# TravisWheelerLab/BATH

Hardware: AMD Instinct MI355X
Metric: DP Gcells/s + residues/s through bathsearch pipeline at 1/2/4/8 MI355X (higher is better)
Workload: dtype u8/i16 integer scores (SSV: exact binary16), f32 Forward

## Files before the change

### bath_amd/__init__.py

```python
import ctypes as C
import os
import subprocess

import numpy as np

_HERE = os.path.dirname(os.path.abspath(__file__))
_ROOT = os.path.dirname(_HERE)
LIB_PATH = os.environ.get("BATH_HIP_LIBRARY") or os.path.join(_HERE, "libbathhip.so")

OK, ERANGE, ENORESULT = 0, 16, 19
KP, K, NEVPARAM = 29, 20, 8
LOGSUM_TABLE, LOGSUM_EXACT, LOGSUM_TABLE_SERIAL, LOGSUM_CONTEXT = 0, 1, 2, 3
LOGSUM_ODDS = 4
ENSEMBLE_SERIAL, ENSEMBLE_STREAMS_HOST, ENSEMBLE_STREAMS_DEVICE = 0, 1, 2
ENSEMBLE_MODES = {"serial": ENSEMBLE_SERIAL, "streams": ENSEMBLE_STREAMS_HOST, "device": ENSEMBLE_STREAMS_DEVICE}
ENS_SAMPLES = 200
ENS_OK, ENS_IMPOSSIBLE, ENS_STEP_CAP, ENS_SEG_OVERFLOW = 0, 1, 2, 3
ENS_REGION_OK, ENS_REGION_NO_TRACES = 0, 1

DNA_SYMS = "ACGT-RYMKSWHBVDN*~"
AMINO_SYMS = "ACDEFGHIKLMNPQRSTVWY-BJZOUX*~"


class BathError(RuntimeError):
# ... 134 lines not shown


class Fs5Result(C.Structure):
    _fields_ = [("fwdsc", C.c_float), ("bcksc", C.c_float), ("oasc", C.c_float), ("null2", C.c_float * KP)]


_vp, _u8p, _f32p, _i32p, _i64p = C.c_void_p, C.POINTER(C.c_uint8), C.POINTER(C.c_float), C.POINTER(C.c_int32), C.POINTER(C.c_int64)
ABI = {
    "bath_hmmfile_count": (C.c_int, [C.c_char_p]),
    "bath_hmmfile_read": (C.c_int, [C.c_char_p, C.c_int, C.POINTER(C.POINTER(_Hmm))]),
    "bath_hmm_destroy": (None, [C.POINTER(_Hmm)]),
    "bath_gencode_basic": (C.c_int, [C.c_int, _u8p]),
    "bath_profile_config": (C.c_int, [C.POINTER(_Hmm), C.c_int, C.POINTER(C.POINTER(_Profile))]),
    "bath_profile_destroy": (None, [C.POINTER(_Profile)]),
    "bath_fs_profile_config": (C.c_int, [C.POINTER(_Hmm), _u8p, C.c_int, C.c_int, C.POINTER(C.POINTER(_FsProfile))]),
    "bath_fs_profile_destroy": (None, [C.POINTER(_FsProfile)]),
    "bath_hip_init": (C.c_int, [C.c_int, C.POINTER(_vp)]),
    "bath_hip_finalize": (None, [_vp]),
    "bath_hip_last_error": (C.c_char_p, [_vp]),
    "bath_hip_synchronize": (C.c_int, [_vp]),
    "bath_hip_stream": (_vp, [_vp]),
    "bath_hip_set_fs_strict": (C.c_int, [_vp, C.c_int]),
    "bath_hip_set_fs_serial": (C.c_int, [_vp, C.c_int]),
    "bath_hip_set_fs_odds": (C.c_int, [_vp, C.c_int]),
    "bath_hip_set_fs5_odds": (C.c_int, [_vp, C.c_int]),
    "bath_hip_set_fs_ensemble": (C.c_int, [_vp, C.c_int]),
    "bath_hip_fs_ensemble_counters": (C.c_int, [_vp, _i64p, _i64p, _i64p]),
    "bath_hip_set_std_ensemble": (C.c_int, [_vp, C.c_int]),
    "bath_hip_std_ensemble_counters": (C.c_int, [_vp, _i64p, _i64p, _i64p]),
    "bath_hip_std_region_ensembles": (C.c_int, [_vp, _vp, _vp, _i32p, C.c_uint32, _i32p, _i32p, _i32p, C.c_int64, _i64p, _i32p, _f32p, C.c_int64, _i64p]),
    "bath_selftest_std_ensemble": (C.c_int, [C.c_int, C.c_int, _f32p, _f32p, C.c_float, C.c_float, C.c_float, _u8p, C.c_int, _f32p, _f32p, C.c_uint32, _i32p, _i32p,
                                             _i32p, C.c_int, _i32p, _f32p, _i32p, C.c_int, _i32p]),
    "bath_selftest_std_ens_walk": (C.c_int, [C.c_int, _f32p, C.c_float, C.c_float, C.c_float, C.c_int, _f32p, _f32p, C.c_uint32, _i32p, _i32p, C.c_int, _i32p]),
    "bath_hip_fs5_region_ensembles": (C.c_int, [_vp, _vp, _vp, C.c_uint32, _i32p, _i32p, _i32p, C.c_int64, _i64p, _i32p, C.c_int64, _i64p]),
    "bath_selftest_fs_ensemble_seeded": (C.c_int, [C.c_int, _f32p, C.c_float, C.c_float, C.c_float, C.c_int, C.c_int, _f32p, _f32p, C.c_uint32, _i32p, C.c_int, _i32p]),
    "bath_selftest_fs_ensemble_streams": (C.c_int, [C.c_int, _f32p, C.c_float, C.c_float, C.c_float, C.c_int, C.c_int, _f32p, _f32p, C.c_uint32,
                                                    _i32p, _i32p, _i32p, C.c_int, _i32p, _i32p, C.c_int, _i32p]),
    "bath_selftest_rng_jump": (C.c_int, [C.c_uint32, C.c_uint64, C.POINTER(C.c_uint32)]),
    "bath_selftest_ens_explog": (C.c_int, [C.c_int, _f32p, _f32p, _f32p]),
    "bath_hip_trim": (C.c_int, [_vp]),
    "bath_hip_kernel_times": (C.c_int, [_vp, C.c_int, C.POINTER(KernelTime)]),
    "bath_hip_oprofile_convert": (C.c_int, [_vp, C.POINTER(_Profile), C.POINTER(_vp)]),
    "bath_hip_oprofile_destroy": (None, [_vp]),
    "bath_hip_oprofile_M": (C.c_int, [_vp]),
    "bath_hip_oprofile_scalars": (C.c_int, [_vp, C.c_int, C.POINTER(OProfileScalars)]),
    "bath_hip_oprofile_get_ssv_scores": (C.c_int, [_vp, _u8p]),
# ... 248 lines not shown

    def set_fs5_odds(self, on=True):
        self._check(lib().bath_hip_set_fs5_odds(self._h, 1 if on else 0), "set_fs5_odds")

    def set_fs_ensemble(self, mode):
        self._check(lib().bath_hip_set_fs_ensemble(self._h, ENSEMBLE_MODES.get(mode, mode)), "set_fs_ensemble")

    def fs_ensemble_counters(self):
        a, b, c = C.c_int64(0), C.c_int64(0), C.c_int64(0)
        self._check(lib().bath_hip_fs_ensemble_counters(self._h, C.byref(a), C.byref(b), C.byref(c)), "fs_ensemble_counters")
        return {"bound_fallbacks": a.value, "overflow_fallbacks": b.value, "matrix_bytes_kept": c.value}

    def set_std_ensemble(self, mode):
        self._check(lib().bath_hip_set_std_ensemble(self._h, ENSEMBLE_MODES.get(mode, mode)), "set_std_ensemble")

    def std_ensemble_counters(self):
        a, b, c = C.c_int64(0), C.c_int64(0), C.c_int64(0)
        self._check(lib().bath_hip_std_ensemble_counters(self._h, C.byref(a), C.byref(b), C.byref(c)), "std_ensemble_counters")
        return {"serial_fallbacks": a.value, "twin_fallbacks": b.value, "kernel_regions": c.value}

    def set_fs_serial(self, on):
        self._check(lib().bath_hip_set_fs_serial(self._h, -1 if on is None else (1 if on else 0)), "set_fs_serial")

    @property
    def stream(self):
        return lib().bath_hip_stream(self._h)

    def close(self):
        if getattr(self, "_h", None):
            lib().bath_hip_finalize(self._h)
            self._h = None

    def __del__(self):
        self.close()


class OProfile:

    def __init__(self, ctx, gm):
        h = _vp()
        ctx._check(lib().bath_hip_oprofile_convert(ctx._h, gm._p, C.byref(h)), "oprofile_convert")
        self.ctx, self._h, self.M, self.gm = ctx, h, gm.M, gm
        hmm = getattr(gm, "hmm", None)
        if hmm is not None and hmm.consensus:
            ctx._check(lib().bath_hip_oprofile_set_consensus(h, hmm.consensus.encode()), "oprofile_set_consensus")

# ... 845 lines not shown
```

### bath_amd/csrc/bath_common.hpp

```cpp
#pragma once
#include <set>
#include <atomic>
#include <hip/hip_runtime.h>

#include <cstdint>
#include <chrono>
#include <cstdio>
#include <cstdlib>
#include <cstring>
#include <condition_variable>
#include <functional>
#include <mutex>
#include <string>
#include <thread>
#include <vector>

#include "bath_hip.h"
#include "bath_tilings.hpp"

namespace bath {

inline hipError_t allow_max_lds(const void *fn) {
  static std::mutex mu;
  static std::set<std::pair<int, const void *>> done;
// ... 115 lines not shown

struct bath_hip_ctx;
namespace bath {
extern std::atomic<int> g_ctx_total, g_ctx_internal;
inline int host_contexts() { return g_ctx_total.load() - g_ctx_internal.load(); }
inline void mark_internal(bath_hip_ctx *c);
}
struct bath_hip_ctx {
  int device = 0;
  hipStream_t stream = nullptr;
  hipStream_t tail_stream = nullptr;
  hipStream_t side_stream = nullptr;
  hipEvent_t ev_fork = nullptr, ev_join = nullptr;
  hipStream_t copy_stream = nullptr;
  hipDeviceProp_t prop{};
  int fs_strict = 1;
  int fs_odds = 0;
  int fs5_odds = 0;
  int fs_ensemble = 0;
  std::atomic<int64_t> fs_ens_bound_fallbacks{0}, fs_ens_overflow_fallbacks{0}, fs_ens_bytes_kept{0};
  int std_ensemble = 0;
  std::atomic<int64_t> std_ens_serial_fallbacks{0}, std_ens_twin_fallbacks{0}, std_ens_kernel_regions{0};
  int fs_serial = -1;
  uint64_t tabs_uid = 0;
  const void *tabs_ptr = nullptr;
  uint64_t fsw_pad_uid = 0;
  int orf_tables_id = -1;
  std::string err;
  void set_error(const std::string &m) { err = m; }
  bath::DevBuf scratch[62];
  bath::HostBuf stage[12];
  template <class T> int stage_upload(int slot, void *dst, const T *src, size_t n, hipStream_t s) {
    if (stage[slot].reserve(n * sizeof(T) + 64) != hipSuccess) { set_error("cannot allocate page-locked staging memory"); return BATH_EFAIL; }
    std::memcpy(stage[slot].p, src, n * sizeof(T));
    if (hipMemcpyAsync(dst, stage[slot].p, n * sizeof(T), hipMemcpyHostToDevice, s) != hipSuccess) { set_error("staging upload failed"); return BATH_EFAIL; }
    return BATH_OK;
  }
  bath::HostBuf pinned[4];
  bath::HostBuf results_pinned;
  bath_orf_result *d_records = nullptr;
  int64_t n_records = 0;
  std::vector<bath_orf> orfs;
  std::vector<bath_fs_window> fs_windows;
  bool keep_fwd_rows = false;
  const float *fwd_rows_kept = nullptr;
  const int64_t *fwd_rows_off = nullptr;
// ... 171 lines not shown
```

### bath_amd/csrc/bath_pipeline.hip

```cpp
#include <algorithm>
#include <cmath>
#include <cstring>
#include <cstdlib>
#include <map>
#include <thread>

#include "bath_common.hpp"
#include "bath_kernels.hpp"
#include "bath_launch.hpp"
#include "host_model.hpp"

using namespace bath;

namespace bath {

static const double kLog2 = 0.69314718055994529;

enum { FLAG_VIT_RUN = 1, FLAG_HAS_WIN = 2 };

struct Counters {
  int cand_count, todo_msv, todo_vit, todo_ssvb, todo_vit2, todo_fwd, win_count, overflow;
  int todo_lb, pad_;
  unsigned long long n_orfs, orf_res;
  unsigned long long n_past_msv, n_past_bias, n_past_vit, n_past_fwd;
  unsigned long long pos_past_msv, pos_past_bias, pos_past_vit, pos_past_fwd;
  unsigned long long res_vit, res_fwd;
  unsigned long long res_seen;
};

struct Params {
  double F1, F2, F3, F4;
  int do_bias, fs_pipe, minlen;
  float evparam[BATH_NEVPARAM];
};

template <int NR, int G>
__global__ __launch_bounds__(256, NR <= 76 ? 4 : 1) void ssv_orf_kernel(const uint8_t *__restrict__ aa, const OrfRec *__restrict__ orfs, const int *__restrict__ n_orfs_dev,
                                                      SeqView dna, const int16_t *__restrict__ cost_tab, int row_bytes,
                                                      const int16_t *__restrict__ emit_thresh, int thresh_max,
                                                      Cand cand, int cand_cap, Counters *__restrict__ ctr, int chunk) {
  extern __shared__ __attribute__((aligned(16))) char lds[];
  if (chunk > 0 && (int64_t)blockIdx.x * (blockDim.x >> 6) * chunk * (64 / G) >= (int64_t)*n_orfs_dev) return;
  {
    const int n32 = kSsvRows * row_bytes / 4;
    const uint32_t *src = reinterpret_cast<const uint32_t *>(cost_tab);
// ... 284 lines not shown
  local_compo_finish(compo, bgf, eo);
}
__device__ void local_compo_finish(float *compo, const float *bgf, float *eo) {
  float sum = 0.f, cc = 0.f;
  for (int x = 0; x < 20; x++) { const float y = compo[x] - cc; const float t = sum + y; cc = (t - sum) - y; sum = t; }
  if (sum != 0.0f) for (int x = 0; x < 20; x++) compo[x] /= sum;
  else for (int x = 0; x < 20; x++) compo[x] = 1.0f / 20.0f;
  for (int x = 0; x < 20; x++) { eo[2 * x] = bgf[x] / bgf[x]; eo[2 * x + 1] = compo[x] / bgf[x]; }
  eo[2 * 20] = eo[2 * 20 + 1] = 1.0f; eo[2 * 27] = eo[2 * 27 + 1] = 1.0f; eo[2 * 28] = eo[2 * 28 + 1] = 1.0f;
  const int mem[6][2] = {{2, 11}, {7, 9}, {3, 13}, {8, 8}, {1, 1}, {-1, -1}};
  for (int dx = 0; dx < 6; dx++) {
    float n0 = 0.f, n1 = 0.f, den = 0.f;
    if (dx == 5) { for (int y = 0; y < 20; y++) { n0 += bgf[y]; n1 += compo[y]; den += bgf[y]; } }
    else {
      const int a = min(mem[dx][0], mem[dx][1]), b = max(mem[dx][0], mem[dx][1]);
      n0 += bgf[a]; n1 += compo[a]; den += bgf[a];
      if (b != a) { n0 += bgf[b]; n1 += compo[b]; den += bgf[b]; }
    }
    eo[2 * (21 + dx)] = den > 0.f ? n0 / den : 0.f;
    eo[2 * (21 + dx) + 1] = den > 0.f ? n1 / den : 0.f;
  }
}

__global__ void post_vit_kernel(Cand cand, int cand_cap, Counters *__restrict__ ctr, Params p, int32_t *__restrict__ todo_lb, int32_t *__restrict__ todo_fwd) {
  const int ncand = min(ctr->cand_count, cand_cap);
  for (int c = blockIdx.x * blockDim.x + threadIdx.x; c < ncand; c += gridDim.x * blockDim.x) {
    if (cand.stage[c] != 2) continue;
    const int L = cand.len[c];
    if (cand.flags[c] & FLAG_VIT_RUN) {
      const float seqsc = (float)((double)(cand.vfsc[c] - cand.filtersc[c]) / kLog2);
      const double P = d_gumbel_surv(seqsc, p.evparam[2], p.evparam[3]);
      cand.P[c] = P;
      if (P > p.F2) { cand.kminmax[2 * c] = 1 << 30; cand.kminmax[2 * c + 1] = 0; continue; }
    }
    atomicAdd(&ctr->n_past_vit, 1ull); atomicAdd(&ctr->pos_past_vit, (unsigned long long)L * 3ull);
    if (p.do_bias && cand.kminmax[2 * c] <= cand.kminmax[2 * c + 1]) {
      cand.flags[c] |= FLAG_HAS_WIN;
      todo_lb[atomicAdd(&ctr->todo_lb, 1)] = c;
      continue;
    }
    cand.stage[c] = 3;
    todo_fwd[atomicAdd(&ctr->todo_fwd, 1)] = c; atomicAdd(&ctr->res_fwd, (unsigned long long)L);
  }
}

__global__ void compo_terms_kernel(const float *__restrict__ bgf, int base_b, float scale_b, float *__restrict__ terms ) {
  const int x = blockIdx.x, sc = threadIdx.x;
  const float lo = ((float)base_b - (float)sc) / scale_b;
  terms[x * 256 + sc] = bgf[x] * expf(lo);
}

__global__ __launch_bounds__(64) void local_compo_kernel(Cand cand, const Counters *__restrict__ ctr, int M, const uint8_t *__restrict__ ssv_scores,
                                                         const float *__restrict__ terms, const int32_t *__restrict__ todo_lb, float *__restrict__ compo_out ) {
  const int lane = threadIdx.x, g = lane / 20, x = lane % 20;
  const int ntodo = ctr->todo_lb;
  for (int base = blockIdx.x * 3; base < ntodo; base += gridDim.x * 3) {
    const int job = base + g;
    if (g >= 3 || job >= ntodo) continue;
// ... 40 lines not shown
        const float seqsc = (float)((double)(vfsc - filtersc) / kLog2);
        const double P = d_gumbel_surv(seqsc, p.evparam[2], p.evparam[3]);
        cand.P[c] = P;
        if (P > p.F2) to_fwd = false;
      }
    }
    if (to_fwd) { cand.stage[c] = 3; todo_fwd[atomicAdd(&ctr->todo_fwd, 1)] = c; atomicAdd(&ctr->res_fwd, (unsigned long long)L); }
  }
}

__global__ void post_vit2_kernel(Cand cand, Counters *__restrict__ ctr, Params p, const int32_t *__restrict__ todo_vit2, int32_t *__restrict__ todo_fwd) {
  const int ntodo = ctr->todo_vit2;
  for (int job = blockIdx.x * blockDim.x + threadIdx.x; job < ntodo; job += gridDim.x * blockDim.x) {
    const int c = todo_vit2[job];
    const float seqsc = (float)((double)(cand.vfsc[c] - cand.filtersc[c]) / kLog2);
    const double P = d_gumbel_surv(seqsc, p.evparam[2], p.evparam[3]);
    cand.P[c] = P;
    if (P > p.F2) { cand.stage[c] = 2; continue; }
    cand.stage[c] = 3;
    todo_fwd[atomicAdd(&ctr->todo_fwd, 1)] = c; atomicAdd(&ctr->res_fwd, (unsigned long long)cand.len[c]);
  }
}

__global__ void final_kernel(Cand cand, Counters *__restrict__ ctr, Params p, const int32_t *__restrict__ todo_fwd) {
  const int ntodo = ctr->todo_fwd;
  for (int job = blockIdx.x * blockDim.x + threadIdx.x; job < ntodo; job += gridDim.x * blockDim.x) {
    const int c = todo_fwd[job];
    const float seqsc = (float)((double)(cand.fwdsc[c] - cand.filtersc[c]) / kLog2);
    const double P = d_exp_surv(seqsc, p.evparam[4], p.evparam[5]);
    cand.P[c] = P;
    if (P > (p.fs_pipe ? p.F4 : p.F3)) continue;
    cand.stage[c] = 4;
    atomicAdd(&ctr->n_past_fwd, 1ull);
    if (!p.fs_pipe) atomicAdd(&ctr->pos_past_fwd, (unsigned long long)cand.len[c] * 3ull);
  }
}

__global__ void copy_count_kernel(const int *src, int64_t *dst) { *dst = *src; }

}


namespace bath {

static int ssv_classify_host(int v, int tjb, const MsvConsts &c, float *sc) {
  if (tjb + c.tbm + c.tec + c.bias >= 127) return BATH_ENORESULT;
  unsigned xE = (v >= -1 - c.bias) ? 255u : (unsigned)(v + 256);
  if ((int)xE >= 255 - c.bias) { *sc = INFINITY; return (c.base - tjb - c.tbm < 128) ? BATH_ENORESULT : BATH_ERANGE; }
  xE = (xE + (unsigned)(c.base - tjb - c.tbm) - 128u) & 0xffffu;
  if ((int)xE >= 255 - c.bias) { *sc = INFINITY; return BATH_ERANGE; }
// ... 25 lines not shown
  }
}

static int ensure_emit_table(bath_hip_ctx *ctx, const bath_hip_oprofile *om, double F1, int maxlen) {
  std::lock_guard<std::mutex> lock(om->grow_mu);
  if (om->emit_F1 == F1 && om->emit_maxlen >= maxlen && om->d_emit) return BATH_OK;
  std::vector<int16_t> tab;
  build_emit_table(om, F1, maxlen, tab);
  if (om->d_emit) om->retired.push_back(om->d_emit);
  om->d_emit = nullptr;
  BATH_HIP_TRY(ctx, hipMalloc((void **)&om->d_emit, tab.size() * sizeof(int16_t) + 64));
  BATH_HIP_TRY(ctx, hipMemcpy(om->d_emit, tab.data(), tab.size() * sizeof(int16_t), hipMemcpyHostToDevice));
  om->emit_F1 = F1; om->emit_maxlen = maxlen;
  return BATH_OK;
}

static int wave_grid_blocks(bath_hip_ctx *ctx) { return ctx->prop.multiProcessorCount * 8; }

struct PipelineWork {
  Cand cand;
  int cand_cap = 0;
  uint8_t *pool = nullptr;
  int32_t *todo_msv = nullptr, *todo_vit = nullptr, *todo_ssvb = nullptr, *todo_vit2 = nullptr, *todo_fwd = nullptr, *todo_sorted = nullptr;
  int *len_bins = nullptr;
  WindowRec *wins = nullptr;
  int win_cap = 0;
  Counters *ctr = nullptr;
};

template <class T>
static T *carve(char *&p, size_t n) {
  T *r = reinterpret_cast<T *>(p);
  p += (n * sizeof(T) + 255) / 256 * 256;
  return r;
}

static size_t layout(PipelineWork &w, char *base, int cap, int win_cap) {
  char *p = base;
  const size_t n = (size_t)cap;
  w.cand_cap = cap; w.win_cap = std::max(2 * cap, win_cap);
  if (win_cap == 0) {
    static const int forced = [] { const char *e = std::getenv("BATH_HIP_TEST_WINCAP"); return e ? std::atoi(e) : 0; }();
    if (forced > 0) w.win_cap = forced;
  }
  w.ctr = carve<Counters>(p, 1);
  w.cand.window = carve<int64_t>(p, n); w.cand.off = carve<int64_t>(p, n); w.cand.P = carve<double>(p, n);
  w.cand.sf = carve<int32_t>(p, n); w.cand.startj = carve<int32_t>(p, n); w.cand.len = carve<int32_t>(p, n);
  w.cand.msv_status = carve<int32_t>(p, n); w.cand.vit_status = carve<int32_t>(p, n); w.cand.fwd_status = carve<int32_t>(p, n); w.cand.stage = carve<int32_t>(p, n);
  w.cand.flags = carve<int32_t>(p, n); w.cand.kminmax = carve<int32_t>(p, 2 * n);
  w.cand.usc = carve<float>(p, n); w.cand.nullsc = carve<float>(p, n); w.cand.filtersc = carve<float>(p, n);
  w.cand.vfsc = carve<float>(p, n); w.cand.fwdsc = carve<float>(p, n);
  w.cand.v = carve<int16_t>(p, n);
  w.todo_msv = carve<int32_t>(p, n); w.todo_vit = carve<int32_t>(p, n); w.todo_ssvb = carve<int32_t>(p, n);
  w.todo_vit2 = carve<int32_t>(p, n); w.todo_fwd = carve<int32_t>(p, n); w.todo_sorted = carve<int32_t>(p, n);
  w.len_bins = carve<int>(p, 2048);
  w.wins = carve<WindowRec>(p, (size_t)w.win_cap);
  return (size_t)(p - base);
}

}

extern "C" void bath_pipeline_params_default(bath_pipeline_params *p, int fs_pipe) {
  p->F1 = 0.02; p->F2 = 1e-3; p->F3 = 1e-5; p->F4 = 5e-4;
  p->do_biasfilter = 1; p->fs_pipe = fs_pipe; p->min_orf_len = 20; p->ncbi_table = 1;
  p->nres_before = 0;
  p->do_null2 = 1; p->std_pipe = 1; p->strands = BATH_STRAND_BOTH; p->initiator = BATH_INIT_ANY;
  p->inc_by_E = 1; p->seed = 42; p->T = 0.0;
}

extern "C" int bath_hip_pipeline_timings(const bath_hip_ctx *ctx, int max, const char **names, float *ms, int64_t *launches) {
  int n = std::min<int>(max, (int)ctx->timings.size());
  for (int i = 0; i < n; i++) { names[i] = ctx->timings[i].name; ms[i] = ctx->timings[i].ms; launches[i] = ctx->timings[i].launches; }
  return n;
}

namespace bath {
struct FilterState {
  PipelineWork W;
  Counters hc{};
  const uint8_t *d_ssvsc = nullptr;
  const float *d_bgf = nullptr;
  OrfTablesDev tt{};
};
}

__global__ __launch_bounds__(64) void fwd_keep_offsets_kernel(const int32_t *__restrict__ todo, const int *__restrict__ ntodo_dev, const int32_t *__restrict__ len,
                                                              int64_t *__restrict__ off, int64_t cap) {
  const int lane = threadIdx.x, n = *ntodo_dev;
  int64_t base = 0;
  for (int j0 = 0; j0 < n; j0 += 64) {
// ... 5 lines not shown
    if (sid >= 0) off[sid] = (base + incl <= cap) ? base + incl - v : (int64_t)-1;
    base += __shfl(incl, 63, 64);
  }
}

static int cascade_model_ok(bath_hip_ctx *ctx, const bath_hip_oprofile *om) {
  if (om->M <= kCascadeMaxNodes) return BATH_OK;
  ctx->set_error("the filter cascade supports models up to " + std::to_string(kCascadeMaxNodes) + " nodes (this one has " + std::to_string(om->M) + ")");
  return BATH_EINVAL;
}

static int launch_ssv_bath(bath_hip_ctx *ctx, hipStream_t stream, const bath_hip_oprofile *om, const Cand &cand, Counters *ctr, const int32_t *todo, const uint8_t *pool,
                           const uint8_t *ssv_scores, const MsvConsts &mc, double invP, WindowRec *wins, int win_cap);

static int run_filters(bath_hip_ctx *ctx, const bath_hip_oprofile *om, const bath_hip_seqs *dna,
                       const bath_pipeline_params *prm, bath_pipeline_stats *stats,
                       const bath_orf_result **results, int64_t *n_results, FilterState *state) {
  if (!ctx || !om || !dna || !prm) return BATH_EINVAL;
  if (cascade_model_ok(ctx, om) != BATH_OK) return BATH_EINVAL;
  BATH_HIP_TRY(ctx, hipSetDevice(ctx->device));
  if (n_results) *n_results = 0;
  if (results) *results = nullptr;
  if (stats) std::memset(stats, 0, sizeof *stats);
  const int64_t nwin = dna->n;
  if (nwin == 0) return BATH_OK;
  const int M = om->M;
  const int max_orf = dna->maxlen / 3 + 1;
  int st = om->ensure_len_tables(max_orf);
  if (st != BATH_OK) return st;

  OrfTablesDev tt{};
  if (prm->strands < 0 || prm->strands > 2 || prm->initiator < 0 || prm->initiator > 2) { ctx->set_error("bath_pipeline_params: strands / initiator out of range"); return BATH_EINVAL; }
  if ((st = orf_tables_upload(ctx, prm->ncbi_table, &tt, prm->initiator)) != BATH_OK) return st;
  if ((st = ensure_emit_table(ctx, om, prm->F1, max_orf)) != BATH_OK) return st;
  DevBuf &b_tabs = ctx->scratch[8], &b_work = ctx->scratch[9];
  const size_t ssv_bytes = (size_t)(M + 1) * kKp;
  const size_t tabs_bytes = 8192 + ssv_bytes + 256 + 20 * 4 + 256;
  if (tabs_bytes > b_tabs.cap) ctx->tabs_uid = 0;
  BATH_HIP_TRY(ctx, b_tabs.reserve(tabs_bytes));
  char *tp = b_tabs.as<char>();
  const int16_t *d_emit = om->d_emit;
  uint8_t *d_ssvsc = reinterpret_cast<uint8_t *>(tp); tp += (ssv_bytes + 255) / 256 * 256;
  float *d_bgf = reinterpret_cast<float *>(tp);
  if (ctx->tabs_uid != om->uid || ctx->tabs_ptr != b_tabs.p) {
    std::vector<uint8_t> ssv_scores(ssv_bytes, 0);
    bath_hip_oprofile_get_ssv_scores(om, ssv_scores.data());
// ... 109 lines not shown
      hipLaunchKernelGGL(classify_kernel, dim3(dec_blocks), dim3(256), 0, ctx->stream, W.cand, W.cand_cap, W.ctr, om->lt.d_tjb, mc, W.todo_msv);
      BATH_HIP_TRY(ctx, hipGetLastError());
      if ((st = launch_msv_wave(ctx, om, cv, W.todo_msv, cap, W.cand.usc, W.cand.msv_status, &W.ctr->todo_msv, !few_msv)) != BATH_OK) return st;
      BATH_HIP_TRY(ctx, hipEventRecord(ev[e++], ctx->stream));
      hipLaunchKernelGGL(f1_bias_kernel, dim3(dec_blocks), dim3(256), 0, ctx->stream, W.cand, W.cand_cap, W.ctr, P, W.pool, M, f1t, W.todo_vit, W.todo_ssvb);
      BATH_HIP_TRY(ctx, hipGetLastError());
      BATH_HIP_TRY(ctx, hipEventRecord(ev[e++], ctx->stream));
    }
    wa.d_filtersc = W.cand.filtersc; wa.d_ssv_scores = d_ssvsc; wa.d_wins = W.wins; wa.d_win_count = &W.ctr->win_count; wa.win_cap = W.win_cap;
    wa.d_kminmax = W.cand.kminmax;
    auto launch_ssvb = [&](hipStream_t stream) -> int {
      return launch_ssv_bath(ctx, stream, om, W.cand, W.ctr, W.todo_ssvb, W.pool, d_ssvsc, mc, invP_f1, W.wins, W.win_cap);
    };
    bool ssvb_done = false;
    if (vit_lane_supported(om) && !few_cands) {
      if ((st = launch_vit_sorted(ctx, om, cv, W.todo_vit, cap, &W.ctr->todo_vit, W.cand.len, W.len_bins, W.todo_sorted, W.cand.vfsc, W.cand.vit_status, &wa,
                                  launch_ssvb)) != BATH_OK) return st;
      ssvb_done = true;
    } else if ((st = launch_vit_wave(ctx, om, cv, W.todo_vit, cap, W.cand.vfsc, W.cand.vit_status, &wa, &W.ctr->todo_vit)) != BATH_OK) return st;
    BATH_HIP_TRY(ctx, hipEventRecord(ev[e++], ctx->stream));
    if (!ssvb_done && (st = launch_ssvb(ctx->stream)) != BATH_OK) return st;
    BATH_HIP_TRY(ctx, hipGetLastError());
    BATH_HIP_TRY(ctx, hipEventRecord(ev[e++], ctx->stream));
    hipLaunchKernelGGL(post_vit_kernel, dim3(dec_blocks), dim3(256), 0, ctx->stream, W.cand, W.cand_cap, W.ctr, P, W.todo_msv , W.todo_fwd);
    if (P.do_bias) {
      DevBuf &b_compo = ctx->scratch[36];
      BATH_HIP_TRY(ctx, b_compo.reserve((size_t)20 * 256 * 4 + (size_t)W.cand_cap * 20 * 4 + 256));
      float *d_terms = b_compo.as<float>(), *d_compo = d_terms + 20 * 256;
      hipLaunchKernelGGL(compo_terms_kernel, dim3(20), dim3(256), 0, ctx->stream, d_bgf, (int)om->base_b, om->scale_b, d_terms);
      hipLaunchKernelGGL(local_compo_kernel, dim3(16384), dim3(64), 0, ctx->stream, W.cand, W.ctr, M, d_ssvsc, d_terms, W.todo_msv, d_compo);
      hipLaunchKernelGGL(post_vit_local_kernel, dim3(std::max(1, dec_blocks)), dim3(64), 0, ctx->stream, W.cand, W.ctr, P, W.pool, M, d_bgf, d_compo,
                         om->lt.d_p1, om->lt.d_lt1, om->lt.d_lt2, W.todo_msv, W.todo_vit2, W.todo_fwd);
    }
    BATH_HIP_TRY(ctx, hipGetLastError());
    if ((st = launch_vit_wave(ctx, om, cv, W.todo_vit2, cap, W.cand.vfsc, W.cand.vit_status, nullptr, &W.ctr->todo_vit2)) != BATH_OK) return st;
    hipLaunchKernelGGL(post_vit2_kernel, dim3(64), dim3(256), 0, ctx->stream, W.cand, W.ctr, P, W.todo_vit2, W.todo_fwd);
    BATH_HIP_TRY(ctx, hipGetLastError());
    BATH_HIP_TRY(ctx, hipEventRecord(ev[e++], ctx->stream));
    ctx->fwd_rows_kept = nullptr; ctx->fwd_rows_off = nullptr;
    float *d_keep = nullptr; int64_t *d_keep_off = nullptr;
    if (ctx->keep_fwd_rows) {
      constexpr int64_t kKeepFloats = (int64_t)8 << 20;
      DevBuf &b_rows = ctx->scratch[38], &b_roff = ctx->scratch[39];
      BATH_HIP_TRY(ctx, b_rows.reserve((size_t)kKeepFloats * sizeof(float) + 64)); BATH_HIP_TRY(ctx, b_roff.reserve((size_t)cap * sizeof(int64_t) + 64));
      d_keep = b_rows.as<float>(); d_keep_off = b_roff.as<int64_t>();
      hipLaunchKernelGGL(fwd_keep_offsets_kernel, dim3(1), dim3(64), 0, ctx->stream, W.todo_fwd, &W.ctr->todo_fwd, W.cand.len, d_keep_off, kKeepFloats);
      BATH_HIP_TRY(ctx, hipGetLastError());
    }
    if ((st = launch_fwd_wave(ctx, om, cv, W.todo_fwd, cap, W.cand.fwdsc, W.cand.fwd_status, &W.ctr->todo_fwd, d_keep, d_keep_off)) != BATH_OK) return st;
    if (d_keep) { ctx->fwd_rows_kept = d_keep; ctx->fwd_rows_off = d_keep_off; }
    hipLaunchKernelGGL(final_kernel, dim3(dec_blocks), dim3(256), 0, ctx->stream, W.cand, W.ctr, P, W.todo_fwd);
    BATH_HIP_TRY(ctx, hipGetLastError());
    BATH_HIP_TRY(ctx, hipEventRecord(ev[e++], ctx->stream));

    BATH_HIP_TRY(ctx, hipMemcpyAsync(&hc, W.ctr, sizeof(Counters), hipMemcpyDeviceToHost, ctx->stream));
    BATH_HIP_TRY(ctx, hipStreamSynchronize(ctx->stream));
    if (hc.overflow || hc.cand_count > cap || hc.win_count > W.win_cap) {
      if (attempt >= 4) { ctx->set_error("candidate / window buffers overflowed repeatedly"); return BATH_EMEM; }
      if (hc.overflow || hc.cand_count > cap) cap = std::max<int64_t>(cap * 2, (int64_t)hc.cand_count + 1024);
      if (hc.win_count > W.win_cap) win_need = hc.win_count + hc.win_count / 4 + 1024;
      continue;
    }
    static const char *names[] = {"translate_orfs", "ssv_f1", "classify_msv", "f1_bias", "viterbi_windows", "ssv_windows", "post_vit", "forward_final"};
    const int64_t launches[] = {4, 1, msv_stage ? 1 : 2, msv_stage ? 0 : 1, 4, 1, 3, 2};
    ctx->timings.clear();
    for (int i = 0; i + 1 < e; i++) {
      float ms = 0.f;
      BATH_HIP_TRY(ctx, hipEventElapsedTime(&ms, ev[i], ev[i + 1]));
      ctx->timings.push_back(StageTiming{names[i], ms, launches[i]});
    }
    break;
  }

  if (stats) {
    stats->nres = nres; stats->n_orfs = (int64_t)hc.n_orfs;
    stats->n_past_msv = (int64_t)hc.n_past_msv; stats->n_past_bias = (int64_t)hc.n_past_bias;
    stats->n_past_vit = (int64_t)hc.n_past_vit; stats->n_past_fwd = (int64_t)hc.n_past_fwd;
    stats->pos_past_msv = (int64_t)hc.pos_past_msv; stats->pos_past_bias = (int64_t)hc.pos_past_bias;
    stats->pos_past_vit = (int64_t)hc.pos_past_vit; stats->pos_past_fwd = (int64_t)hc.pos_past_fwd;
    stats->cells_msv = (int64_t)(hc.orf_res - hc.res_seen) * M; stats->cells_vit = (int64_t)hc.res_vit * M; stats->cells_fwd = (int64_t)hc.res_fwd * M;
  }

  if (results) {
    bath_orf_result *d_rec = nullptr;
    int64_t nrec = 0;
    if (dna->n > (int64_t)UINT32_MAX || dna->maxlen / 3 >= (1 << 28)) { ctx->set_error("block too large for the ORF records' sort key (2^32 windows, 805 Mnt per window)"); return BATH_ERANGE; }
    if ((st = build_orf_records(ctx, W.cand, hc.cand_count, dna->is_part ? dna->first_window : 0, &d_rec, &nrec)) != BATH_OK) return st;
// ... 71 lines not shown
  }
  BATH_HIP_TRY(ctx, hipSetDevice(ctx->device));
  int st = om->ensure_len_tables(dna->maxlen / 3 + 1);
  if (st != BATH_OK) return st;
  if ((st = ensure_emit_table(ctx, om, prm->F1, dna->maxlen / 3 + 1)) != BATH_OK) return st;
  while ((int)ctx->lanes.size() < K) {
    bath_hip_ctx *lane = nullptr;
    if ((st = bath_hip_init(ctx->device, &lane)) != BATH_OK) { ctx->set_error("cannot create a pipeline lane"); return st; }
    mark_internal(lane);
    const char *pe = std::getenv("BATH_HIP_LANE_PRIO");
    if (!(pe && pe[0] == '0')) {
      int lo = 0, hi = 0;
      if (hipDeviceGetStreamPriorityRange(&lo, &hi) == hipSuccess && lo != hi) {
        (void)hipStreamDestroy(lane->stream);
        const char *te = std::getenv("BATH_HIP_TAIL_PRIO");
        const bool tails = te && te[0] == '1';
        const int prio = tails ? (ctx->lanes.empty() ? std::min(lo, hi + 1) : lo) : (ctx->lanes.empty() ? hi : lo);
        if (hipStreamCreateWithPriority(&lane->stream, hipStreamNonBlocking, prio) != hipSuccess) { ctx->set_error("hipStreamCreateWithPriority"); return BATH_EFAIL; }
        if (tails && hipStreamCreateWithPriority(&lane->tail_stream, hipStreamNonBlocking, hi) != hipSuccess) { ctx->set_error("hipStreamCreateWithPriority"); return BATH_EFAIL; }
      }
    }
    ctx->lanes.push_back(lane);
  }
  for (bath_hip_ctx *lane : ctx->lanes) { lane->fs_strict = ctx->fs_strict; lane->fs_odds = ctx->fs_odds; lane->fs5_odds = ctx->fs5_odds; }
  if ((st = ensure_parts(ctx, dna, K)) != BATH_OK) return st;
  std::vector<bath_pipeline_stats> pst((size_t)K);
  std::vector<const bath_orf_result *> pres((size_t)K, nullptr);
  std::vector<int64_t> pn((size_t)K, 0);
  std::vector<int> rc((size_t)K, BATH_OK);
  states->assign((size_t)K, FilterState{});
  if (!ctx->ev_lanes) BATH_HIP_TRY(ctx, hipEventCreateWithFlags(&ctx->ev_lanes, hipEventDisableTiming));
  BATH_HIP_TRY(ctx, hipEventRecord(ctx->ev_lanes, ctx->stream));
  for (int k = 0; k < K; k++) BATH_HIP_TRY(ctx, hipStreamWaitEvent(ctx->lanes[(size_t)k]->stream, ctx->ev_lanes, 0));
  if (!ctx->lane_pool) ctx->lane_pool = new LanePool();
  ctx->lane_pool->run(K, [&](int k) {
    bath_hip_ctx *lane = ctx->lanes[(size_t)k];
    rc[(size_t)k] = run_filters(lane, om, dna->parts[(size_t)k], prm, &pst[(size_t)k], results ? &pres[(size_t)k] : nullptr, &pn[(size_t)k], &(*states)[(size_t)k]);
    if (rc[(size_t)k] == BATH_OK) rc[(size_t)k] = after(k, lane, dna->parts[(size_t)k], (*states)[(size_t)k]);
  });
  for (int k = 0; k < K; k++)
    if (rc[(size_t)k] != BATH_OK) { ctx->set_error(ctx->lanes[(size_t)k]->err); return rc[(size_t)k]; }

  bath_pipeline_stats tot{};
  int64_t ntot = 0;
  for (int k = 0; k < K; k++) {
    const bath_pipeline_stats &a = pst[(size_t)k];
    tot.nres += a.nres; tot.n_orfs += a.n_orfs; tot.n_past_msv += a.n_past_msv; tot.n_past_bias += a.n_past_bias; tot.n_past_vit += a.n_past_vit;
    tot.n_past_fwd += a.n_past_fwd; tot.pos_past_msv += a.pos_past_msv; tot.pos_past_bias += a.pos_past_bias; tot.pos_past_vit += a.pos_past_vit;
    tot.pos_past_fwd += a.pos_past_fwd; tot.cells_msv += a.cells_msv; tot.cells_vit += a.cells_vit; tot.cells_fwd += a.cells_fwd;
    ntot += pn[(size_t)k];
  }
  if (stats) *stats = tot;
  if (results) {
    BATH_HIP_TRY(ctx, ctx->results_pinned.reserve((size_t)std::max<int64_t>(ntot, 1) * sizeof(bath_orf_result)));
    bath_orf_result *dst = ctx->results_pinned.as<bath_orf_result>();
    int64_t at = 0;
    for (int k = 0; k < K; k++) {
      bath_hip_ctx *lane = ctx->lanes[(size_t)k];
      const int64_t nk = pn[(size_t)k];
      if (nk > 0) BATH_HIP_TRY(ctx, hipMemcpyAsync(dst + at, lane->d_records, (size_t)nk * sizeof(bath_orf_result), hipMemcpyDeviceToHost, lane->stream));
      at += nk;
    }
    for (int k = 0; k < K; k++) BATH_HIP_TRY(ctx, hipStreamSynchronize(ctx->lanes[(size_t)k]->stream));
    *results = dst;
  }
  if (n_results) *n_results = ntot;
  ctx->timings.clear();
  for (int k = 0; k < K; k++) {
    const std::vector<StageTiming> &t = ctx->lanes[(size_t)k]->timings;
    for (size_t i = 0; i < t.size(); i++) {
      if (k == 0) ctx->timings.push_back(t[i]);
      else if (i < ctx->timings.size()) { ctx->timings[i].ms += t[i].ms; ctx->timings[i].launches += t[i].launches; }
    }
  }
  return BATH_OK;
}

extern "C" int bath_hip_pipeline_filters_repeat(bath_hip_ctx *ctx, const bath_hip_oprofile *om, const bath_hip_seqs *dna,
                                                const bath_pipeline_params *prm, int reps, bath_pipeline_stats *stats) {
  std::vector<FilterState> states;
  int st = run_filters_lanes(ctx, om, dna, prm, stats, nullptr, nullptr, &states,
                             [&](int, bath_hip_ctx *lane, const bath_hip_seqs *part, const FilterState &) {
                               for (int r = 1; r < reps; r++) {
                                 bath_pipeline_stats s2{};
                                 int64_t n2 = 0;
                                 const int rc = run_filters(lane, om, part, prm, &s2, nullptr, &n2, nullptr);
                                 if (rc != BATH_OK) return rc;
                               }
                               return (int)BATH_OK;
                             });
  return st;
// ... 465 lines not shown
```

### bath_amd/csrc/bath_profile.hip

```cpp
#include <atomic>
#include <cctype>
#include <cmath>
#include <cstring>

#include "bath_common.hpp"
#include "host_model.hpp"

using namespace bath;

namespace bath {

static const double kLog2 = 0.69314718055994529;

double gumbel_surv(double x, double mu, double lambda) {
  double ey = -std::exp(-lambda * (x - mu));
  if (std::fabs(ey) < 5e-9) return -ey;
  return 1.0 - std::exp(ey);
}
double gumbel_invsurv(double p, double mu, double lambda) {
  double lp = (p < 5e-9) ? (std::pow(p, p) - 1) / p : std::log(-1. * std::log(1 - p));
  return mu - lp / lambda;
}
double exp_surv(double x, double mu, double lambda) { return (x < mu) ? 1.0 : std::exp(-lambda * (x - mu)); }

// ... 155 lines not shown
  return BATH_OK;
}

extern "C" void *bath_hip_stream(bath_hip_ctx *ctx) { return (void *)ctx->stream; }
extern "C" int bath_hip_kernel_times(bath_hip_ctx *ctx, int max, bath_kernel_time *out) {
  if (!ctx || !out) return 0;
  int n = 0;
  for (const bath_hip_ctx *c : {(const bath_hip_ctx *)ctx, (const bath_hip_ctx *)ctx->aux, (const bath_hip_ctx *)ctx->aux2, (const bath_hip_ctx *)ctx->aux3}) {
    if (!c) continue;
    for (const bath::KernelSpan &k : c->spans) {
      float ms = 0.f;
      if (hipEventSynchronize(k.b) != hipSuccess || hipEventElapsedTime(&ms, k.a, k.b) != hipSuccess) continue;
      int i = 0;
      while (i < n && out[i].name != k.name) i++;
      if (i == n) { if (n == max) continue; out[n++] = bath_kernel_time{k.name, 0.f, 0, 0.0, 0.0}; }
      out[i].ms += ms; out[i].launches++; out[i].cells += k.cells; out[i].bytes += k.bytes;
    }
  }
  return n;
}
extern "C" int bath_hip_set_fs_serial(bath_hip_ctx *ctx, int on) {
  if (!ctx) return BATH_EINVAL;
  ctx->fs_serial = on < 0 ? -1 : (on ? 1 : 0);
  return BATH_OK;
}

extern "C" int bath_hip_set_fs_strict(bath_hip_ctx *ctx, int on) {
  if (!ctx) return BATH_EINVAL;
  ctx->fs_strict = on ? 1 : 0;
  if (!on && ctx->aux3) { bath_hip_finalize(ctx->aux3); ctx->aux3 = nullptr; }
  for (bath_hip_ctx *l : ctx->lanes) l->fs_strict = ctx->fs_strict;
  return BATH_OK;
}

extern "C" int bath_hip_set_fs_odds(bath_hip_ctx *ctx, int on) {
  if (!ctx) return BATH_EINVAL;
  ctx->fs_odds = on ? 1 : 0;
  for (bath_hip_ctx *l : ctx->lanes) l->fs_odds = ctx->fs_odds;
  return BATH_OK;
}

extern "C" int bath_hip_set_fs5_odds(bath_hip_ctx *ctx, int on) {
  if (!ctx) return BATH_EINVAL;
  ctx->fs5_odds = on ? 1 : 0;
  for (bath_hip_ctx *l : ctx->lanes) l->fs5_odds = ctx->fs5_odds;
  return BATH_OK;
// ... 452 lines not shown
```

### include/bath_hip.h

```cpp
#ifndef BATH_HIP_H
#define BATH_HIP_H

#include <stdint.h>
#include <stddef.h>

#ifdef __cplusplus
extern "C" {
#endif

#define BATH_OK          0
#define BATH_EFAIL       1
#define BATH_EMEM        5
#define BATH_EFORMAT     7
#define BATH_EINVAL     11
#define BATH_ERANGE     16
#define BATH_ENORESULT  19
#define BATH_ENODEVICE  40

#define BATH_KP_AMINO   29
#define BATH_K_AMINO    20
#define BATH_KP_DNA     18
#define BATH_NEVPARAM    8
#define BATH_FTAU        4
#define BATH_FLAMBDA     5
// ... 49 lines not shown
int  bath_profile_config(const bath_hmm *hmm, int L, bath_profile **ret);
void bath_profile_destroy(bath_profile *gm);
int  bath_fs_profile_config(const bath_hmm *hmm, const uint8_t basic[64], int codon_lengths, int L_amino,
                            bath_fs_profile **ret);
void bath_fs_profile_destroy(bath_fs_profile *gm);

int         bath_hip_init(int device, bath_hip_ctx **ctx);
void        bath_hip_finalize(bath_hip_ctx *ctx);
const char *bath_hip_last_error(const bath_hip_ctx *ctx);
int         bath_hip_synchronize(bath_hip_ctx *ctx);
int         bath_hip_trim(bath_hip_ctx *ctx);
void       *bath_hip_stream(bath_hip_ctx *ctx);
int         bath_hip_set_fs_strict(bath_hip_ctx *ctx, int on);
int         bath_hip_set_fs_odds(bath_hip_ctx *ctx, int on);
int         bath_hip_set_fs5_odds(bath_hip_ctx *ctx, int on);
#define BATH_ENSEMBLE_SERIAL 0
#define BATH_ENSEMBLE_STREAMS_HOST 1
#define BATH_ENSEMBLE_STREAMS_DEVICE 2
int         bath_hip_set_fs_ensemble(bath_hip_ctx *ctx, int mode);
int         bath_hip_fs_ensemble_counters(bath_hip_ctx *ctx, int64_t *bound_fallbacks, int64_t *overflow_fallbacks, int64_t *matrix_bytes_kept);
int         bath_hip_set_std_ensemble(bath_hip_ctx *ctx, int mode);
int         bath_hip_std_ensemble_counters(bath_hip_ctx *ctx, int64_t *serial_fallbacks, int64_t *twin_fallbacks, int64_t *kernel_regions);
int         bath_hip_set_fs_serial(bath_hip_ctx *ctx, int on);

int  bath_hip_oprofile_convert(bath_hip_ctx *ctx, const bath_profile *gm, bath_hip_oprofile **ret);
void bath_hip_oprofile_destroy(bath_hip_oprofile *om);
int  bath_hip_oprofile_set_consensus(bath_hip_oprofile *om, const char *consensus);
int  bath_hip_oprofile_M(const bath_hip_oprofile *om);

typedef struct {
  uint8_t tbm_b, tec_b, tjb_b, base_b, bias_b;
  float   scale_b;
  int16_t xw[4][2];
  float   scale_w;
  int16_t base_w, ddbound_w;
  float   xf[4][2];
} bath_oprofile_scalars;
int  bath_hip_oprofile_scalars(const bath_hip_oprofile *om, int L, bath_oprofile_scalars *out);
int  bath_hip_oprofile_get_ssv_scores(const bath_hip_oprofile *om, uint8_t *arr);
int  bath_hip_oprofile_get_vit(const bath_hip_oprofile *om, int16_t *rw, int16_t *tw);
int  bath_hip_oprofile_get_fwd(const bath_hip_oprofile *om, float *rf, float *tf);

int     bath_hip_seqs_create(bath_hip_ctx *ctx, const uint8_t *dsq, const int64_t *offsets, int64_t n, bath_hip_seqs **ret);
void    bath_hip_seqs_destroy(bath_hip_seqs *sq);
int64_t bath_hip_seqs_count(const bath_hip_seqs *sq);
int  bath_hip_seqs_set_context(bath_hip_seqs *sq, const int32_t *context);
// ... 302 lines not shown
```

Measured before the change: 200.5 billion.

## Speculatively run Forward on all post-Viterbi survivors on side stream

Result: faster. 203.9 billion (median of 6 runs) (+1.7%).

```diff
diff --git a/bath_amd/__init__.py b/bath_amd/__init__.py
--- a/bath_amd/__init__.py
+++ b/bath_amd/__init__.py
@@ -180,6 +180,8 @@
     "bath_hip_stream": (_vp, [_vp]),
     "bath_hip_set_fs_strict": (C.c_int, [_vp, C.c_int]),
     "bath_hip_set_fs_serial": (C.c_int, [_vp, C.c_int]),
+    "bath_hip_set_fwd_spec": (C.c_int, [_vp, C.c_int]),
+    "bath_hip_pipeline_fwd_spec_counts": (C.c_int, [_vp, _i64p, _i64p, _i64p]),
     "bath_hip_set_fs_odds": (C.c_int, [_vp, C.c_int]),
     "bath_hip_set_fs5_odds": (C.c_int, [_vp, C.c_int]),
     "bath_hip_set_fs_ensemble": (C.c_int, [_vp, C.c_int]),
@@ -474,6 +476,14 @@
     def set_fs_serial(self, on):
         self._check(lib().bath_hip_set_fs_serial(self._h, -1 if on is None else (1 if on else 0)), "set_fs_serial")
 
+    def set_fwd_spec(self, on=True):
+        self._check(lib().bath_hip_set_fwd_spec(self._h, 1 if on else 0), "set_fwd_spec")
+
+    def fwd_spec_counts(self):
+        a, b, c = C.c_int64(0), C.c_int64(0), C.c_int64(0)
+        self._check(lib().bath_hip_pipeline_fwd_spec_counts(self._h, C.byref(a), C.byref(b), C.byref(c)), "pipeline_fwd_spec_counts")
+        return {"todo_spec": a.value, "todo_fwd": b.value, "todo_vit2": c.value}
+
     @property
     def stream(self):
         return lib().bath_hip_stream(self._h)
diff --git a/bath_amd/csrc/bath_common.hpp b/bath_amd/csrc/bath_common.hpp
--- a/bath_amd/csrc/bath_common.hpp
+++ b/bath_amd/csrc/bath_common.hpp
@@ -161,6 +161,8 @@
   int std_ensemble = 0;
   std::atomic<int64_t> std_ens_serial_fallbacks{0}, std_ens_twin_fallbacks{0}, std_ens_kernel_regions{0};
   int fs_serial = -1;
+  int fwd_spec = 1;
+  int64_t fwd_spec_counts[3] = {0, 0, 0};
   uint64_t tabs_uid = 0;
   const void *tabs_ptr = nullptr;
   uint64_t fsw_pad_uid = 0;
diff --git a/bath_amd/csrc/bath_pipeline.hip b/bath_amd/csrc/bath_pipeline.hip
--- a/bath_amd/csrc/bath_pipeline.hip
+++ b/bath_amd/csrc/bath_pipeline.hip
@@ -20,7 +20,7 @@
 
 struct Counters {
   int cand_count, todo_msv, todo_vit, todo_ssvb, todo_vit2, todo_fwd, win_count, overflow;
-  int todo_lb, pad_;
+  int todo_lb, todo_spec;
   unsigned long long n_orfs, orf_res;
   unsigned long long n_past_msv, n_past_bias, n_past_vit, n_past_fwd;
   unsigned long long pos_past_msv, pos_past_bias, pos_past_vit, pos_past_fwd;
@@ -351,7 +351,8 @@
   }
 }
 
-__global__ void post_vit_kernel(Cand cand, int cand_cap, Counters *__restrict__ ctr, Params p, int32_t *__restrict__ todo_lb, int32_t *__restrict__ todo_fwd) {
+__global__ void post_vit_kernel(Cand cand, int cand_cap, Counters *__restrict__ ctr, Params p, int32_t *__restrict__ todo_lb, int32_t *__restrict__ todo_fwd,
+                                int32_t *__restrict__ todo_spec) {
   const int ncand = min(ctr->cand_count, cand_cap);
   for (int c = blockIdx.x * blockDim.x + threadIdx.x; c < ncand; c += gridDim.x * blockDim.x) {
     if (cand.stage[c] != 2) continue;
@@ -363,6 +364,7 @@
       if (P > p.F2) { cand.kminmax[2 * c] = 1 << 30; cand.kminmax[2 * c + 1] = 0; continue; }
     }
     atomicAdd(&ctr->n_past_vit, 1ull); atomicAdd(&ctr->pos_past_vit, (unsigned long long)L * 3ull);
+    if (todo_spec) todo_spec[atomicAdd(&ctr->todo_spec, 1)] = c;
     if (p.do_bias && cand.kminmax[2 * c] <= cand.kminmax[2 * c + 1]) {
       cand.flags[c] |= FLAG_HAS_WIN;
       todo_lb[atomicAdd(&ctr->todo_lb, 1)] = c;
@@ -449,10 +451,12 @@
   }
 }
 
-__global__ void final_kernel(Cand cand, Counters *__restrict__ ctr, Params p, const int32_t *__restrict__ todo_fwd) {
+__global__ void final_kernel(Cand cand, Counters *__restrict__ ctr, Params p, const int32_t *__restrict__ todo_fwd,
+                             const float *__restrict__ spec_sc, const int32_t *__restrict__ spec_status) {
   const int ntodo = ctr->todo_fwd;
   for (int job = blockIdx.x * blockDim.x + threadIdx.x; job < ntodo; job += gridDim.x * blockDim.x) {
     const int c = todo_fwd[job];
+    if (spec_sc) { cand.fwdsc[c] = spec_sc[c]; cand.fwd_status[c] = spec_status[c]; }
     const float seqsc = (float)((double)(cand.fwdsc[c] - cand.filtersc[c]) / kLog2);
     const double P = d_exp_surv(seqsc, p.evparam[4], p.evparam[5]);
     cand.P[c] = P;
@@ -524,6 +528,8 @@
   int cand_cap = 0;
   uint8_t *pool = nullptr;
   int32_t *todo_msv = nullptr, *todo_vit = nullptr, *todo_ssvb = nullptr, *todo_vit2 = nullptr, *todo_fwd = nullptr, *todo_sorted = nullptr;
+  int32_t *todo_spec = nullptr, *spec_status = nullptr;
+  float *spec_sc = nullptr;
   int *len_bins = nullptr;
   WindowRec *wins = nullptr;
   int win_cap = 0;
@@ -555,6 +561,7 @@
   w.cand.v = carve<int16_t>(p, n);
   w.todo_msv = carve<int32_t>(p, n); w.todo_vit = carve<int32_t>(p, n); w.todo_ssvb = carve<int32_t>(p, n);
   w.todo_vit2 = carve<int32_t>(p, n); w.todo_fwd = carve<int32_t>(p, n); w.todo_sorted = carve<int32_t>(p, n);
+  w.todo_spec = carve<int32_t>(p, n); w.spec_status = carve<int32_t>(p, n); w.spec_sc = carve<float>(p, n);
   w.len_bins = carve<int>(p, 2048);
   w.wins = carve<WindowRec>(p, (size_t)w.win_cap);
   return (size_t)(p - base);
@@ -568,6 +575,14 @@
   p->nres_before = 0;
   p->do_null2 = 1; p->std_pipe = 1; p->strands = BATH_STRAND_BOTH; p->initiator = BATH_INIT_ANY;
   p->inc_by_E = 1; p->seed = 42; p->T = 0.0;
+}
+
+extern "C" int bath_hip_pipeline_fwd_spec_counts(const bath_hip_ctx *ctx, int64_t *todo_spec, int64_t *todo_fwd, int64_t *todo_vit2) {
+  if (!ctx) return BATH_EINVAL;
+  if (todo_spec) *todo_spec = ctx->fwd_spec_counts[0];
+  if (todo_fwd) *todo_fwd = ctx->fwd_spec_counts[1];
+  if (todo_vit2) *todo_vit2 = ctx->fwd_spec_counts[2];
+  return BATH_OK;
 }
 
 extern "C" int bath_hip_pipeline_timings(const bath_hip_ctx *ctx, int max, const char **names, float *ms, int64_t *launches) {
@@ -619,6 +634,7 @@
   if (n_results) *n_results = 0;
   if (results) *results = nullptr;
   if (stats) std::memset(stats, 0, sizeof *stats);
+  ctx->fwd_spec_counts[0] = ctx->fwd_spec_counts[1] = ctx->fwd_spec_counts[2] = 0;
   const int64_t nwin = dna->n;
   if (nwin == 0) return BATH_OK;
   const int M = om->M;
@@ -774,7 +790,20 @@
     if (!ssvb_done && (st = launch_ssvb(ctx->stream)) != BATH_OK) return st;
     BATH_HIP_TRY(ctx, hipGetLastError());
     BATH_HIP_TRY(ctx, hipEventRecord(ev[e++], ctx->stream));
-    hipLaunchKernelGGL(post_vit_kernel, dim3(dec_blocks), dim3(256), 0, ctx->stream, W.cand, W.cand_cap, W.ctr, P, W.todo_msv , W.todo_fwd);
+    const bool fwd_spec = ctx->fwd_spec && !ctx->keep_fwd_rows;
+    hipLaunchKernelGGL(post_vit_kernel, dim3(dec_blocks), dim3(256), 0, ctx->stream, W.cand, W.cand_cap, W.ctr, P, W.todo_msv , W.todo_fwd,
+                       fwd_spec ? W.todo_spec : nullptr);
+    BATH_HIP_TRY(ctx, hipGetLastError());
+    struct SideDrain { bath_hip_ctx *c; bool armed; ~SideDrain() { if (armed) (void)hipStreamSynchronize(c->side_stream); } } side_drain{ctx, false};
+    if (fwd_spec) {
+      if ((st = fs_fork(ctx)) != BATH_OK) return st;
+      side_drain.armed = true;
+      hipStream_t main_stream = ctx->stream;
+      ctx->stream = ctx->side_stream;
+      st = launch_fwd_wave(ctx, om, cv, W.todo_spec, cap, W.spec_sc, W.spec_status, &W.ctr->todo_spec);
+      ctx->stream = main_stream;
+      if (st != BATH_OK) return st;
+    }
     if (P.do_bias) {
       DevBuf &b_compo = ctx->scratch[36];
       BATH_HIP_TRY(ctx, b_compo.reserve((size_t)20 * 256 * 4 + (size_t)W.cand_cap * 20 * 4 + 256));
@@ -799,9 +828,13 @@
       hipLaunchKernelGGL(fwd_keep_offsets_kernel, dim3(1), dim3(64), 0, ctx->stream, W.todo_fwd, &W.ctr->todo_fwd, W.cand.len, d_keep_off, kKeepFloats);
       BATH_HIP_TRY(ctx, hipGetLastError());
     }
-    if ((st = launch_fwd_wave(ctx, om, cv, W.todo_fwd, cap, W.cand.fwdsc, W.cand.fwd_status, &W.ctr->todo_fwd, d_keep, d_keep_off)) != BATH_OK) return st;
+    if (fwd_spec) {
+      if ((st = fs_join(ctx)) != BATH_OK) return st;
+      side_drain.armed = false;
+    } else if ((st = launch_fwd_wave(ctx, om, cv, W.todo_fwd, cap, W.cand.fwdsc, W.cand.fwd_status, &W.ctr->todo_fwd, d_keep, d_keep_off)) != BATH_OK) return st;
     if (d_keep) { ctx->fwd_rows_kept = d_keep; ctx->fwd_rows_off = d_keep_off; }
-    hipLaunchKernelGGL(final_kernel, dim3(dec_blocks), dim3(256), 0, ctx->stream, W.cand, W.ctr, P, W.todo_fwd);
+    hipLaunchKernelGGL(final_kernel, dim3(dec_blocks), dim3(256), 0, ctx->stream, W.cand, W.ctr, P, W.todo_fwd, fwd_spec ? W.spec_sc : nullptr,
+                       fwd_spec ? W.spec_status : nullptr);
     BATH_HIP_TRY(ctx, hipGetLastError());
     BATH_HIP_TRY(ctx, hipEventRecord(ev[e++], ctx->stream));
 
@@ -814,7 +847,9 @@
       continue;
     }
     static const char *names[] = {"translate_orfs", "ssv_f1", "classify_msv", "f1_bias", "viterbi_windows", "ssv_windows", "post_vit", "forward_final"};
-    const int64_t launches[] = {4, 1, msv_stage ? 1 : 2, msv_stage ? 0 : 1, 4, 1, 3, 2};
+    const int64_t n_post_vit = 3 + (P.do_bias ? 3 : 0) + (fwd_spec ? 1 : 0), n_fwd_final = fwd_spec ? 1 : 2 + (ctx->keep_fwd_rows ? 1 : 0);
+    const int64_t launches[] = {4, 1, msv_stage ? 1 : 2, msv_stage ? 0 : 1, 4, 1, n_post_vit, n_fwd_final};
+    ctx->fwd_spec_counts[0] = hc.todo_spec; ctx->fwd_spec_counts[1] = hc.todo_fwd; ctx->fwd_spec_counts[2] = hc.todo_vit2;
     ctx->timings.clear();
     for (int i = 0; i + 1 < e; i++) {
       float ms = 0.f;
@@ -932,7 +967,7 @@
     }
     ctx->lanes.push_back(lane);
   }
-  for (bath_hip_ctx *lane : ctx->lanes) { lane->fs_strict = ctx->fs_strict; lane->fs_odds = ctx->fs_odds; lane->fs5_odds = ctx->fs5_odds; }
+  for (bath_hip_ctx *lane : ctx->lanes) { lane->fs_strict = ctx->fs_strict; lane->fs_odds = ctx->fs_odds; lane->fs5_odds = ctx->fs5_odds; lane->fwd_spec = ctx->fwd_spec; }
   if ((st = ensure_parts(ctx, dna, K)) != BATH_OK) return st;
   std::vector<bath_pipeline_stats> pst((size_t)K);
   std::vector<const bath_orf_result *> pres((size_t)K, nullptr);
@@ -976,7 +1011,9 @@
   }
   if (n_results) *n_results = ntot;
   ctx->timings.clear();
+  for (int64_t &n : ctx->fwd_spec_counts) n = 0;
   for (int k = 0; k < K; k++) {
+    for (int i = 0; i < 3; i++) ctx->fwd_spec_counts[i] += ctx->lanes[(size_t)k]->fwd_spec_counts[i];
     const std::vector<StageTiming> &t = ctx->lanes[(size_t)k]->timings;
     for (size_t i = 0; i < t.size(); i++) {
       if (k == 0) ctx->timings.push_back(t[i]);
diff --git a/bath_amd/csrc/bath_profile.hip b/bath_amd/csrc/bath_profile.hip
--- a/bath_amd/csrc/bath_profile.hip
+++ b/bath_amd/csrc/bath_profile.hip
@@ -201,6 +201,12 @@
 extern "C" int bath_hip_set_fs_serial(bath_hip_ctx *ctx, int on) {
   if (!ctx) return BATH_EINVAL;
   ctx->fs_serial = on < 0 ? -1 : (on ? 1 : 0);
+  return BATH_OK;
+}
+
+extern "C" int bath_hip_set_fwd_spec(bath_hip_ctx *ctx, int on) {
+  if (!ctx) return BATH_EINVAL;
+  ctx->fwd_spec = on ? 1 : 0;
   return BATH_OK;
 }
 
diff --git a/include/bath_hip.h b/include/bath_hip.h
--- a/include/bath_hip.h
+++ b/include/bath_hip.h
@@ -95,6 +95,8 @@
 int         bath_hip_set_std_ensemble(bath_hip_ctx *ctx, int mode);
 int         bath_hip_std_ensemble_counters(bath_hip_ctx *ctx, int64_t *serial_fallbacks, int64_t *twin_fallbacks, int64_t *kernel_regions);
 int         bath_hip_set_fs_serial(bath_hip_ctx *ctx, int on);
+int         bath_hip_set_fwd_spec(bath_hip_ctx *ctx, int on);
+int         bath_hip_pipeline_fwd_spec_counts(const bath_hip_ctx *ctx, int64_t *todo_spec, int64_t *todo_fwd, int64_t *todo_vit2);
 
 int  bath_hip_oprofile_convert(bath_hip_ctx *ctx, const bath_profile *gm, bath_hip_oprofile **ret);
 void bath_hip_oprofile_destroy(bath_hip_oprofile *om);
```
